# jramapuram/BYOL

Hardware: NVIDIA H100
Metric: images/sec (higher is better)
Workload: dtype bf16

## Files before the change

### byol_b200/csrc/common.cuh

```cuda
#pragma once
#include <cuda.h>
#include <cuda_bf16.h>
#include <cuda_runtime.h>
#include <stdint.h>

namespace byol {

typedef __nv_bfloat16 bf16;

void set_last_error(const char* fmt, ...);
int check_launch(const char* what);

static constexpr int kMaxDevices = 64;
int device_slot();
int device_sm_count();

int smem_opt_in(const void* kernel, int bytes, const char* what);

int tmap_bf16(CUtensorMap* tm, const void* base, int rank, const uint64_t* dims, const uint64_t* byte_strides,
              const uint32_t* box, CUtensorMapSwizzle swizzle, const char* what);
int tmap_2d(CUtensorMap* tm, const void* base, uint64_t rows, uint64_t cols, uint64_t ld, uint32_t box_rows,
            uint32_t box_cols, const char* what);

struct Fix128 {
// ... 74 lines not shown
      ::byol::set_last_error(__VA_ARGS__);        \
      return -1;                                  \
    }                                             \
  } while (0)

__device__ __forceinline__ uint32_t smem_u32(const void* p) {
  return (uint32_t)__cvta_generic_to_shared(p);
}

__device__ __forceinline__ bool elect_one() {
  uint32_t pred = 0;
  asm volatile(
      "{\n"
      ".reg .b32 %%rx;\n"
      ".reg .pred %%px;\n"
      "elect.sync %%rx|%%px, %1;\n"
      "@%%px mov.s32 %0, 1;\n"
      "}\n"
      : "+r"(pred)
      : "r"(0xffffffffu));
  return pred != 0;
}

__device__ __forceinline__ void nesterov_update(float& w, float& buf, float& grad, float lr, float wd, float mu) {
  const float g = __fadd_rn(grad, __fmul_rn(wd, w));
  buf = __fadd_rn(__fmul_rn(mu, buf), g);
  const float d = __fadd_rn(g, __fmul_rn(mu, buf));
  w = __fsub_rn(w, __fmul_rn(lr, d));
  grad = 0.f;
}

__device__ __forceinline__ float warp_sum(float v) {
#pragma unroll
  for (int o = 16; o > 0; o >>= 1) v += __shfl_xor_sync(0xffffffffu, v, o);
  return v;
}

__device__ __forceinline__ void mbar_init(uint64_t* bar, uint32_t count) {
  asm volatile("mbarrier.init.shared::cta.b64 [%0], %1;" ::"r"(smem_u32(bar)), "r"(count) : "memory");
}
__device__ __forceinline__ void fence_mbar_init() {
  asm volatile("fence.mbarrier_init.release.cluster;" ::: "memory");
}
__device__ __forceinline__ void mbar_arrive(uint64_t* bar) {
  asm volatile("mbarrier.arrive.shared::cta.b64 _, [%0];" ::"r"(smem_u32(bar)) : "memory");
}
__device__ __forceinline__ void mbar_arrive_expect_tx(uint64_t* bar, uint32_t bytes) {
  asm volatile("mbarrier.arrive.expect_tx.shared::cta.b64 _, [%0], %1;" ::"r"(smem_u32(bar)), "r"(bytes)
               : "memory");
}
__device__ __forceinline__ bool mbar_try_wait(uint64_t* bar, uint32_t parity) {
  uint32_t ok;
  asm volatile(
      "{\n"
      ".reg .pred p;\n"
      "mbarrier.try_wait.parity.shared::cta.b64 p, [%1], %2;\n"
      "selp.u32 %0, 1, 0, p;\n"
      "}\n"
      : "=r"(ok)
      : "r"(smem_u32(bar)), "r"(parity)
      : "memory");
  return ok != 0;
}
__device__ __forceinline__ void mbar_wait(uint64_t* bar, uint32_t parity) {
  uint32_t spins = 0;
  while (!mbar_try_wait(bar, parity)) {
    if (++spins > (1u << 28)) __trap();
  }
}

__device__ __forceinline__ void fence_proxy_async_smem() {
  asm volatile("fence.proxy.async.shared::cta;" ::: "memory");
}

__device__ __forceinline__ void cp_async16_zfill(uint32_t dst_smem, const void* src, bool valid) {
  uint32_t sz = valid ? 16u : 0u;
  asm volatile("cp.async.cg.shared.global [%0], [%1], 16, %2;" ::"r"(dst_smem), "l"(src), "r"(sz) : "memory");
}
__device__ __forceinline__ void cp_async_commit() { asm volatile("cp.async.commit_group;" ::: "memory"); }
template <int N>
__device__ __forceinline__ void cp_async_wait() {
  asm volatile("cp.async.wait_group %0;" ::"n"(N) : "memory");
}

__device__ __forceinline__ void tma_prefetch_desc(const CUtensorMap* tmap) {
  asm volatile("prefetch.tensormap [%0];" ::"l"(tmap) : "memory");
}
__device__ __forceinline__ void tma_load_2d(uint32_t dst_smem, const CUtensorMap* tmap, uint64_t* bar, int c0,
                                            int c1) {
  asm volatile(
      "cp.async.bulk.tensor.2d.shared::cluster.global.mbarrier::complete_tx::bytes [%0], [%1, {%3, %4}], [%2];"
      ::"r"(dst_smem), "l"(tmap), "r"(smem_u32(bar)), "r"(c0), "r"(c1)
      : "memory");
}

__device__ __forceinline__ void tma_store_2d(const CUtensorMap* tmap, uint32_t src_smem, int c0, int c1) {
  asm volatile("cp.async.bulk.tensor.2d.global.shared::cta.bulk_group [%0, {%2, %3}], [%1];" ::"l"(tmap),
               "r"(src_smem), "r"(c0), "r"(c1)
               : "memory");
}
__device__ __forceinline__ void tma_store_commit() { asm volatile("cp.async.bulk.commit_group;" ::: "memory"); }
__device__ __forceinline__ void tma_store_wait_read() {
  asm volatile("cp.async.bulk.wait_group.read 0;" ::: "memory");
}
__device__ __forceinline__ void tma_store_wait_read1() {
  asm volatile("cp.async.bulk.wait_group.read 1;" ::: "memory");
}
__device__ __forceinline__ void tma_store_wait_all() { asm volatile("cp.async.bulk.wait_group 0;" ::: "memory"); }

__device__ __forceinline__ void wg_fence() { asm volatile("wgmma.fence.sync.aligned;" ::: "memory"); }
__device__ __forceinline__ void wg_commit() { asm volatile("wgmma.commit_group.sync.aligned;" ::: "memory"); }
template <int N>
__device__ __forceinline__ void wg_wait() {
  asm volatile("wgmma.wait_group.sync.aligned %0;" ::"n"(N) : "memory");
}
template <int R>
__device__ __forceinline__ void wg_fence_acc(float (&d)[R]) {
#pragma unroll
  for (int i = 0; i < R; ++i) asm volatile("" : "+f"(d[i])::"memory");
}

template <int N, int TA, int TB>
__device__ __forceinline__ void wgmma_bf16(float (&d)[N / 2], uint64_t adesc, uint64_t bdesc, uint32_t accumulate) {
  static_assert(N == 32 || N == 64 || N == 128 || N == 192 || N == 256, "wgmma_bf16: unsupported N");
  if constexpr (N == 32) {
    asm volatile(
        "{\n.reg .pred p;\nsetp.ne.b32 p, %18, 0;\n"
        "wgmma.mma_async.sync.aligned.m64n32k16.f32.bf16.bf16 {%0, %1, %2, %3, %4, %5, %6, %7, %8, %9, %10, %11, %12, %13, %14, %15}, %16, %17, p, 1, 1, %19, %20;\n}\n"
        : "+f"(d[0]), "+f"(d[1]), "+f"(d[2]), "+f"(d[3]), "+f"(d[4]), "+f"(d[5]), "+f"(d[6]), "+f"(d[7]), "+f"(d[8]), "+f"(d[9]), "+f"(d[10]), "+f"(d[11]), "+f"(d[12]), "+f"(d[13]), "+f"(d[14]), "+f"(d[15])
        : "l"(adesc), "l"(bdesc), "r"(accumulate), "n"(TA), "n"(TB));
  }
  if constexpr (N == 64) {
    asm volatile(
        "{\n.reg .pred p;\nsetp.ne.b32 p, %34, 0;\n"
        "wgmma.mma_async.sync.aligned.m64n64k16.f32.bf16.bf16 {%0, %1, %2, %3, %4, %5, %6, %7, %8, %9, %10, %11, %12, %13, %14, %15, %16, %17, %18, %19, %20, %21, %22, %23, %24, %25, %26, %27, %28, %29, %30, %31}, %32, %33, p, 1, 1, %35, %36;\n}\n"
        : "+f"(d[0]), "+f"(d[1]), "+f"(d[2]), "+f"(d[3]), "+f"(d[4]), "+f"(d[5]), "+f"(d[6]), "+f"(d[7]), "+f"(d[8]), "+f"(d[9]), "+f"(d[10]), "+f"(d[11]), "+f"(d[12]), "+f"(d[13]), "+f"(d[14]), "+f"(d[15]), "+f"(d[16]), "+f"(d[17]), "+f"(d[18]), "+f"(d[19]), "+f"(d[20]), "+f"(d[21]), "+f"(d[22]), "+f"(d[23]), "+f"(d[24]), "+f"(d[25]), "+f"(d[26]), "+f"(d[27]), "+f"(d[28]), "+f"(d[29]), "+f"(d[30]), "+f"(d[31])
        : "l"(adesc), "l"(bdesc), "r"(accumulate), "n"(TA), "n"(TB));
  }
  if constexpr (N == 128) {
    asm volatile(
        "{\n.reg .pred p;\nsetp.ne.b32 p, %66, 0;\n"
        "wgmma.mma_async.sync.aligned.m64n128k16.f32.bf16.bf16 {%0, %1, %2, %3, %4, %5, %6, %7, %8, %9, %10, %11, %12, %13, %14, %15, %16, %17, %18, %19, %20, %21, %22, %23, %24, %25, %26, %27, %28, %29, %30, %31, %32, %33, %34, %35, %36, %37, %38, %39, %40, %41, %42, %43, %44, %45, %46, %47, %48, %49, %50, %51, %52, %53, %54, %55, %56, %57, %58, %59, %60, %61, %62, %63}, %64, %65, p, 1, 1, %67, %68;\n}\n"
        : "+f"(d[0]), "+f"(d[1]), "+f"(d[2]), "+f"(d[3]), "+f"(d[4]), "+f"(d[5]), "+f"(d[6]), "+f"(d[7]), "+f"(d[8]), "+f"(d[9]), "+f"(d[10]), "+f"(d[11]), "+f"(d[12]), "+f"(d[13]), "+f"(d[14]), "+f"(d[15]), "+f"(d[16]), "+f"(d[17]), "+f"(d[18]), "+f"(d[19]), "+f"(d[20]), "+f"(d[21]), "+f"(d[22]), "+f"(d[23]), "+f"(d[24]), "+f"(d[25]), "+f"(d[26]), "+f"(d[27]), "+f"(d[28]), "+f"(d[29]), "+f"(d[30]), "+f"(d[31]), "+f"(d[32]), "+f"(d[33]), "+f"(d[34]), "+f"(d[35]), "+f"(d[36]), "+f"(d[37]), "+f"(d[38]), "+f"(d[39]), "+f"(d[40]), "+f"(d[41]), "+f"(d[42]), "+f"(d[43]), "+f"(d[44]), "+f"(d[45]), "+f"(d[46]), "+f"(d[47]), "+f"(d[48]), "+f"(d[49]), "+f"(d[50]), "+f"(d[51]), "+f"(d[52]), "+f"(d[53]), "+f"(d[54]), "+f"(d[55]), "+f"(d[56]), "+f"(d[57]), "+f"(d[58]), "+f"(d[59]), "+f"(d[60]), "+f"(d[61]), "+f"(d[62]), "+f"(d[63])
        : "l"(adesc), "l"(bdesc), "r"(accumulate), "n"(TA), "n"(TB));
  }
  if constexpr (N == 192) {
    asm volatile(
        "{\n.reg .pred p;\nsetp.ne.b32 p, %98, 0;\n"
        "wgmma.mma_async.sync.aligned.m64n192k16.f32.bf16.bf16 {%0, %1, %2, %3, %4, %5, %6, %7, %8, %9, %10, %11, %12, %13, %14, %15, %16, %17, %18, %19, %20, %21, %22, %23, %24, %25, %26, %27, %28, %29, %30, %31, %32, %33, %34, %35, %36, %37, %38, %39, %40, %41, %42, %43, %44, %45, %46, %47, %48, %49, %50, %51, %52, %53, %54, %55, %56, %57, %58, %59, %60, %61, %62, %63, %64, %65, %66, %67, %68, %69, %70, %71, %72, %73, %74, %75, %76, %77, %78, %79, %80, %81, %82, %83, %84, %85, %86, %87, %88, %89, %90, %91, %92, %93, %94, %95}, %96, %97, p, 1, 1, %99, %100;\n}\n"
        : "+f"(d[0]), "+f"(d[1]), "+f"(d[2]), "+f"(d[3]), "+f"(d[4]), "+f"(d[5]), "+f"(d[6]), "+f"(d[7]), "+f"(d[8]), "+f"(d[9]), "+f"(d[10]), "+f"(d[11]), "+f"(d[12]), "+f"(d[13]), "+f"(d[14]), "+f"(d[15]), "+f"(d[16]), "+f"(d[17]), "+f"(d[18]), "+f"(d[19]), "+f"(d[20]), "+f"(d[21]), "+f"(d[22]), "+f"(d[23]), "+f"(d[24]), "+f"(d[25]), "+f"(d[26]), "+f"(d[27]), "+f"(d[28]), "+f"(d[29]), "+f"(d[30]), "+f"(d[31]), "+f"(d[32]), "+f"(d[33]), "+f"(d[34]), "+f"(d[35]), "+f"(d[36]), "+f"(d[37]), "+f"(d[38]), "+f"(d[39]), "+f"(d[40]), "+f"(d[41]), "+f"(d[42]), "+f"(d[43]), "+f"(d[44]), "+f"(d[45]), "+f"(d[46]), "+f"(d[47]), "+f"(d[48]), "+f"(d[49]), "+f"(d[50]), "+f"(d[51]), "+f"(d[52]), "+f"(d[53]), "+f"(d[54]), "+f"(d[55]), "+f"(d[56]), "+f"(d[57]), "+f"(d[58]), "+f"(d[59]), "+f"(d[60]), "+f"(d[61]), "+f"(d[62]), "+f"(d[63]), "+f"(d[64]), "+f"(d[65]), "+f"(d[66]), "+f"(d[67]), "+f"(d[68]), "+f"(d[69]), "+f"(d[70]), "+f"(d[71]), "+f"(d[72]), "+f"(d[73]), "+f"(d[74]), "+f"(d[75]), "+f"(d[76]), "+f"(d[77]), "+f"(d[78]), "+f"(d[79]), "+f"(d[80]), "+f"(d[81]), "+f"(d[82]), "+f"(d[83]), "+f"(d[84]), "+f"(d[85]), "+f"(d[86]), "+f"(d[87]), "+f"(d[88]), "+f"(d[89]), "+f"(d[90]), "+f"(d[91]), "+f"(d[92]), "+f"(d[93]), "+f"(d[94]), "+f"(d[95])
        : "l"(adesc), "l"(bdesc), "r"(accumulate), "n"(TA), "n"(TB));
  }
  if constexpr (N == 256) {
    asm volatile(
        "{\n.reg .pred p;\nsetp.ne.b32 p, %130, 0;\n"
        "wgmma.mma_async.sync.aligned.m64n256k16.f32.bf16.bf16 {%0, %1, %2, %3, %4, %5, %6, %7, %8, %9, %10, %11, %12, %13, %14, %15, %16, %17, %18, %19, %20, %21, %22, %23, %24, %25, %26, %27, %28, %29, %30, %31, %32, %33, %34, %35, %36, %37, %38, %39, %40, %41, %42, %43, %44, %45, %46, %47, %48, %49, %50, %51, %52, %53, %54, %55, %56, %57, %58, %59, %60, %61, %62, %63, %64, %65, %66, %67, %68, %69, %70, %71, %72, %73, %74, %75, %76, %77, %78, %79, %80, %81, %82, %83, %84, %85, %86, %87, %88, %89, %90, %91, %92, %93, %94, %95, %96, %97, %98, %99, %100, %101, %102, %103, %104, %105, %106, %107, %108, %109, %110, %111, %112, %113, %114, %115, %116, %117, %118, %119, %120, %121, %122, %123, %124, %125, %126, %127}, %128, %129, p, 1, 1, %131, %132;\n}\n"
        : "+f"(d[0]), "+f"(d[1]), "+f"(d[2]), "+f"(d[3]), "+f"(d[4]), "+f"(d[5]), "+f"(d[6]), "+f"(d[7]), "+f"(d[8]), "+f"(d[9]), "+f"(d[10]), "+f"(d[11]), "+f"(d[12]), "+f"(d[13]), "+f"(d[14]), "+f"(d[15]), "+f"(d[16]), "+f"(d[17]), "+f"(d[18]), "+f"(d[19]), "+f"(d[20]), "+f"(d[21]), "+f"(d[22]), "+f"(d[23]), "+f"(d[24]), "+f"(d[25]), "+f"(d[26]), "+f"(d[27]), "+f"(d[28]), "+f"(d[29]), "+f"(d[30]), "+f"(d[31]), "+f"(d[32]), "+f"(d[33]), "+f"(d[34]), "+f"(d[35]), "+f"(d[36]), "+f"(d[37]), "+f"(d[38]), "+f"(d[39]), "+f"(d[40]), "+f"(d[41]), "+f"(d[42]), "+f"(d[43]), "+f"(d[44]), "+f"(d[45]), "+f"(d[46]), "+f"(d[47]), "+f"(d[48]), "+f"(d[49]), "+f"(d[50]), "+f"(d[51]), "+f"(d[52]), "+f"(d[53]), "+f"(d[54]), "+f"(d[55]), "+f"(d[56]), "+f"(d[57]), "+f"(d[58]), "+f"(d[59]), "+f"(d[60]), "+f"(d[61]), "+f"(d[62]), "+f"(d[63]), "+f"(d[64]), "+f"(d[65]), "+f"(d[66]), "+f"(d[67]), "+f"(d[68]), "+f"(d[69]), "+f"(d[70]), "+f"(d[71]), "+f"(d[72]), "+f"(d[73]), "+f"(d[74]), "+f"(d[75]), "+f"(d[76]), "+f"(d[77]), "+f"(d[78]), "+f"(d[79]), "+f"(d[80]), "+f"(d[81]), "+f"(d[82]), "+f"(d[83]), "+f"(d[84]), "+f"(d[85]), "+f"(d[86]), "+f"(d[87]), "+f"(d[88]), "+f"(d[89]), "+f"(d[90]), "+f"(d[91]), "+f"(d[92]), "+f"(d[93]), "+f"(d[94]), "+f"(d[95]), "+f"(d[96]), "+f"(d[97]), "+f"(d[98]), "+f"(d[99]), "+f"(d[100]), "+f"(d[101]), "+f"(d[102]), "+f"(d[103]), "+f"(d[104]), "+f"(d[105]), "+f"(d[106]), "+f"(d[107]), "+f"(d[108]), "+f"(d[109]), "+f"(d[110]), "+f"(d[111]), "+f"(d[112]), "+f"(d[113]), "+f"(d[114]), "+f"(d[115]), "+f"(d[116]), "+f"(d[117]), "+f"(d[118]), "+f"(d[119]), "+f"(d[120]), "+f"(d[121]), "+f"(d[122]), "+f"(d[123]), "+f"(d[124]), "+f"(d[125]), "+f"(d[126]), "+f"(d[127])
        : "l"(adesc), "l"(bdesc), "r"(accumulate), "n"(TA), "n"(TB));
  }
}

template <int N>
__device__ __forceinline__ void acc_store_smem(float* buf, int ld, int row0, int col0, const float (&d)[N / 2]) {
  const int t = threadIdx.x & 127;
  const int r = row0 + (t >> 5) * 16 + ((t & 31) >> 2);
  const int c = col0 + 2 * (t & 3);
// ... 130 lines not shown
```

### byol_b200/csrc/conv_igemm.cu

```cuda
#include <stdarg.h>
#include <stdio.h>
#include <stdlib.h>
#include <string.h>

#include "common.cuh"

namespace byol {

static constexpr int BM = 128;
static constexpr int BK = 64;
static constexpr int A_STAGE_BYTES = BM * 128;
static constexpr int GATHER_LAG = 2;

struct ConvGemmParams {
  const bf16* src;
  void* dst;
  const bf16* resid;
  const uint8_t* resid_mask;
  int resid_up;
  const float* resid_f32;
  const float* bias;
  float* col_sum;
  float* col_sqsum;
  Fix128* fx;
  int Nimg, Hs, Ws, C;
  int Ho, Wo;
  int KH, KW;
  int mul, base, dk, div;
  int M, Ndim, Kg;
  int ldc;
  int num_kb;
  int tiles_n;
  int out_fp32;
  int relu;
  int small_src;
  int local_stats;
  int fold;
  int parity;
  int Hh, Wh;
  int Mc;
  int ncls;
  int cls_list[4];
};

struct TileInfo {
  int m0, n0, nkb;
  int cls_idx, ph, pw, kh0, kw0, nkw;
};

template <bool GROUPED = false>
__device__ __forceinline__ TileInfo tile_info(const ConvGemmParams& p, int tile, int BN_) {
  TileInfo t;
  t.m0 = (tile / p.tiles_n) * BM;
  t.n0 = (tile % p.tiles_n) * BN_;
  t.nkb = p.num_kb;
  t.cls_idx = 0; t.ph = 0; t.pw = 0; t.kh0 = 0; t.kw0 = 0; t.nkw = p.KW;
  if (p.parity) {
    t.cls_idx = t.m0 / p.Mc;
    const int cls = p.cls_list[t.cls_idx];
    t.ph = cls >> 1;
    t.pw = cls & 1;
    t.kh0 = (t.ph + p.base) & 1;
    t.kw0 = (t.pw + p.base) & 1;
    const int nkh = (p.KH - t.kh0 + 1) >> 1;
    t.nkw = (p.KW - t.kw0 + 1) >> 1;
    t.nkb = nkh * t.nkw * (GROUPED ? 1 : p.C / BK);
  }
  return t;
}

template <int BN, int STAGES, bool A_TMA, bool H16 = false>
struct SmemLayout {
  static constexpr int EW = A_TMA ? 8 : 4;
  static constexpr int CPW = (BN / 32) / (EW / 4);
  static constexpr int NBUF = (A_TMA && BN == 128) ? 1 : 2;
  static constexpr int STAGE_PER_WARP = NBUF * 2048;
  static constexpr int B_STAGE_BYTES = BN * 128;
  static constexpr int A_OFF = 0;
  static constexpr int B_OFF = STAGES * A_STAGE_BYTES;
  static constexpr int STAGE_OUT_OFF = B_OFF + STAGES * B_STAGE_BYTES;
  static constexpr int ACC_LD = acc_ld(BN);
  static constexpr int ACC_OFF = STAGE_OUT_OFF + EW * STAGE_PER_WARP;
  static constexpr int OUT_TILE_BYTES = BM * BN * 2;
  static constexpr int BAR_OFF = H16 ? STAGE_OUT_OFF + 2 * OUT_TILE_BYTES : ACC_OFF + BM * ACC_LD * 4;
  static constexpr int NEEDED = BAR_OFF + 256;
  static constexpr int TOTAL = NEEDED + 768;
  static_assert(TOTAL <= 232448, "one CTA per SM: <= 227 KB of dynamic shared memory");
};

static constexpr int IG_THREADS = 17 * 32;

__device__ __forceinline__ void epilogue_bar_sync(int n) { asm volatile("bar.sync 1, %0;" ::"r"(n) : "memory"); }

template <int BN, int STAGES, bool A_TMA, bool GROUPED = false, bool H16 = false>
__global__ void __launch_bounds__(IG_THREADS, 1)
// ... 206 lines not shown
          if (mvalid) {
            float* op = reinterpret_cast<float*>(p.dst) + (int64_t)m * p.ldc + nbase;
            const bool vec = (p.ldc & 3) == 0;
#pragma unroll
            for (int j = 0; j < 32; j += 4) {
              if (vec && nbase + j + 3 < p.Ndim) {
                *reinterpret_cast<float4*>(op + j) = make_float4(v[j], v[j + 1], v[j + 2], v[j + 3]);
              } else {
#pragma unroll
                for (int e = 0; e < 4; ++e)
                  if (nbase + j + e < p.Ndim) op[j + e] = v[j + e];
              }
            }
          }
        } else {
          const uint32_t stage_base = stage_base0 + (uint32_t)sbuf * 2048u;
          if (lane == 0) { if (L::NBUF == 2) tma_store_wait_read1(); else tma_store_wait_read(); }
          __syncwarp();
#pragma unroll
          for (int j = 0; j < 4; ++j) {
            uint4 q;
            q.x = pack_bf16x2(v[8 * j + 0], v[8 * j + 1]);
            q.y = pack_bf16x2(v[8 * j + 2], v[8 * j + 3]);
            q.z = pack_bf16x2(v[8 * j + 4], v[8 * j + 5]);
            q.w = pack_bf16x2(v[8 * j + 6], v[8 * j + 7]);
            const uint32_t off = (uint32_t)lane * 64u + (uint32_t)((j ^ ((lane >> 1) & 3)) << 4);
            asm volatile("st.shared.v4.b32 [%0], {%1, %2, %3, %4};" ::"r"(stage_base + off), "r"(q.x), "r"(q.y),
                         "r"(q.z), "r"(q.w)
                         : "memory");
          }
          fence_proxy_async_smem();
          __syncwarp();
          if (lane == 0) {
            tma_store_2d(&tmapC, stage_base, nbase, mrow0);
            tma_store_commit();
          }
          if (do_stats) stats_narrow(stage_base, lane, rows_valid, cs1[cl], cs2[cl]);
          if (L::NBUF == 2) sbuf ^= 1;
        }
      }
    }
    if (do_stats && stat_n0 >= 0) flush_stats();
    if (local_stats) {
      epilogue_bar_sync(EW * 32);
      for (int i = threadIdx.x; i < 2 * p.Ndim; i += EW * 32) {
        const unsigned long long lo = lstats[2 * i], hi = lstats[2 * i + 1];
        if ((lo | hi) != 0ull) fix_add_words(p.fx + i, lo, (long long)hi);
      }
    }
    if (lane == 0) tma_store_wait_all();
  } else if (!A_TMA && warp >= EW && warp < EW + 4) {
    const int tid = threadIdx.x - 128;
    const int chunk = tid & 7;
    const int row0 = tid >> 3;
    int it = 0;
    const bool fast = GROUPED || ((p.C % BK == 0) && (p.KH * p.KW <= 32) && p.small_src);
    for (int tile = blockIdx.x; tile < num_tiles; tile += gridDim.x) {
      const TileInfo ti = tile_info<GROUPED>(p, tile, BN);
      const int m0 = ti.m0;
      if (!GROUPED && p.fold) {
        uint32_t mask[8];
        int roff[8];
#pragma unroll
        for (int i = 0; i < 8; ++i) {
          const int m = m0 + row0 + 16 * i;
          mask[i] = 0u;
          roff[i] = 0;
          if (m < p.M) {
            const int ow = m % p.Wo;
            const int t = m / p.Wo;
            const int oh = t % p.Ho;
            const int n = t / p.Ho;
            const int bh = oh * p.mul + p.base, bw = ow * p.mul + p.base;
            const int sw = bw + chunk;
            roff[i] = ((n * p.Hs + bh) * p.Ws + sw) * 8;
            if (chunk < p.KW && sw >= 0 && sw < p.Ws)
              for (int kh = 0; kh < p.KH; ++kh)
                if (bh + kh >= 0 && bh + kh < p.Hs) mask[i] |= 1u << kh;
          }
        }
        for (int kb = 0; kb < num_kb; ++kb, ++it) {
          const int s = it % STAGES;
          const uint32_t ph = (it / STAGES) & 1;
          if (it >= GATHER_LAG) {
            cp_async_wait<GATHER_LAG - 1>();
            fence_proxy_async_smem();
            mbar_arrive(&full_bar[(it - GATHER_LAG) % STAGES]);
          }
          mbar_wait(&empty_bar[s], ph ^ 1);
          const int tapoff = kb * p.Ws * 8;
          const uint32_t stage_base = smem_u32(smemA + s * A_STAGE_BYTES);
#pragma unroll
          for (int i = 0; i < 8; ++i) {
            const bool v = (mask[i] >> kb) & 1u;
            const bf16* g = v ? p.src + (roff[i] + tapoff) : p.src;
            cp_async16_zfill(stage_base + sw128_offset(row0 + 16 * i, chunk), g, v);
          }
          cp_async_commit();
        }
      } else if (p.parity) {
        uint32_t mask[8];
        int roff[8];
#pragma unroll
        for (int i = 0; i < 8; ++i) {
          const int mc = m0 + row0 + 16 * i - ti.cls_idx * p.Mc;
          const int b = mc % p.Wh;
          const int t2 = mc / p.Wh;
          const int a = t2 % p.Hh;
          const int n = t2 / p.Hh;
          roff[i] = ((n * p.Hs + a) * p.Ws + b) * p.C;
          mask[i] = 0u;
          int tapi = 0;
          for (int kh = ti.kh0; kh < p.KH; kh += 2)
            for (int kw = ti.kw0; kw < p.KW; kw += 2, ++tapi) {
              const int sh = a + ((ti.ph + p.base - kh) >> 1), sw = b + ((ti.pw + p.base - kw) >> 1);
              if (sh >= 0 && sh < p.Hs && sw >= 0 && sw < p.Ws) mask[i] |= 1u << tapi;
            }
        }
        int kh = ti.kh0, kw = ti.kw0, cc = GROUPED ? ti.n0 : 0, tapi = 0;
        for (int kb = 0; kb < ti.nkb; ++kb, ++it) {
          const int s = it % STAGES;
          const uint32_t ph = (it / STAGES) & 1;
          if (it >= GATHER_LAG) {
            cp_async_wait<GATHER_LAG - 1>();
            fence_proxy_async_smem();
            mbar_arrive(&full_bar[(it - GATHER_LAG) % STAGES]);
          }
          mbar_wait(&empty_bar[s], ph ^ 1);
          const int tapoff = (((ti.ph + p.base - kh) >> 1) * p.Ws + ((ti.pw + p.base - kw) >> 1)) * p.C + cc + chunk * 8;
          const uint32_t stage_base = smem_u32(smemA + s * A_STAGE_BYTES);
#pragma unroll
          for (int i = 0; i < 8; ++i) {
            const bool v = (mask[i] >> tapi) & 1u;
            const bf16* g = v ? p.src + (roff[i] + tapoff) : p.src;
            cp_async16_zfill(stage_base + sw128_offset(row0 + 16 * i, chunk), g, v);
          }
          cp_async_commit();
          if (!GROUPED) cc += BK;
          if (GROUPED || cc >= p.C) {
            if (!GROUPED) cc = 0;
            ++tapi;
            kw += 2;
            if (kw >= p.KW) { kw = ti.kw0; kh += 2; }
          }
        }
      } else if (fast) {
        uint32_t mask[8];
        int roff[8];
#pragma unroll
        for (int i = 0; i < 8; ++i) {
          const int m = m0 + row0 + 16 * i;
          mask[i] = 0u;
          roff[i] = 0;
          if (m < p.M) {
            const int ow = m % p.Wo;
            const int t = m / p.Wo;
            const int oh = t % p.Ho;
            const int n = t / p.Ho;
            const int bh = oh * p.mul + p.base, bw = ow * p.mul + p.base;
            const int sft = p.div == 2 ? 1 : 0;
            roff[i] = ((n * p.Hs + (bh >> sft)) * p.Ws + (bw >> sft)) * p.C;
            int tapi = 0;
            for (int kh = 0; kh < p.KH; ++kh)
              for (int kw = 0; kw < p.KW; ++kw, ++tapi) {
                int sh = bh + kh * p.dk, sw = bw + kw * p.dk;
                bool ok = sh >= 0 && sw >= 0;
                if (p.div == 2) { ok = ok && ((sh | sw) & 1) == 0; sh >>= 1; sw >>= 1; }
                if (ok && sh < p.Hs && sw < p.Ws) mask[i] |= 1u << tapi;
              }
          }
        }
        int kh = 0, kw = 0, cc = GROUPED ? ti.n0 : 0, tapi = 0;
        for (int kb = 0; kb < num_kb; ++kb, ++it) {
          const int s = it % STAGES;
          const uint32_t ph = (it / STAGES) & 1;
          if (it >= GATHER_LAG) {
            cp_async_wait<GATHER_LAG - 1>();
            fence_proxy_async_smem();
            mbar_arrive(&full_bar[(it - GATHER_LAG) % STAGES]);
          }
          mbar_wait(&empty_bar[s], ph ^ 1);
          const int tapoff = (p.div == 2 ? -((kh >> 1) * p.Ws + (kw >> 1)) : (kh * p.Ws + kw) * p.dk) * p.C + cc +
                             chunk * 8;
          const uint32_t stage_base = smem_u32(smemA + s * A_STAGE_BYTES);
#pragma unroll
          for (int i = 0; i < 8; ++i) {
            const bool v = (mask[i] >> tapi) & 1u;
            const bf16* g = v ? p.src + (roff[i] + tapoff) : p.src;
            cp_async16_zfill(stage_base + sw128_offset(row0 + 16 * i, chunk), g, v);
          }
          cp_async_commit();
          if (!GROUPED) cc += BK;
          if (GROUPED || cc >= p.C) {
            if (!GROUPED) cc = 0;
            ++tapi;
            if (++kw == p.KW) { kw = 0; ++kh; }
          }
        }
      } else if (!GROUPED) {
        int bh[8], bw[8];
        int64_t ioff[8];
#pragma unroll
        for (int i = 0; i < 8; ++i) {
          int m = m0 + row0 + 16 * i;
          if (m < p.M) {
            int ow = m % p.Wo;
            int t = m / p.Wo;
            int oh = t % p.Ho;
            int n = t / p.Ho;
            bh[i] = oh * p.mul + p.base;
            bw[i] = ow * p.mul + p.base;
            ioff[i] = (int64_t)n * p.Hs * p.Ws * p.C;
          } else {
            bh[i] = -(1 << 28);
            bw[i] = -(1 << 28);
            ioff[i] = 0;
          }
        }
        for (int kb = 0; kb < num_kb; ++kb, ++it) {
          const int s = it % STAGES;
          const uint32_t ph = (it / STAGES) & 1;
          if (it >= GATHER_LAG) {
            cp_async_wait<GATHER_LAG - 1>();
            fence_proxy_async_smem();
            mbar_arrive(&full_bar[(it - GATHER_LAG) % STAGES]);
          }
          mbar_wait(&empty_bar[s], ph ^ 1);
          const int k0 = kb * BK + chunk * 8;
          const bool kvalid = k0 < p.Kg;
          const int tap = k0 / p.C;
          const int cc = k0 - tap * p.C;
          const int kh = tap / p.KW;
          const int kw = tap - kh * p.KW;
          const int dh = kh * p.dk, dw = kw * p.dk;
          const uint32_t stage_base = smem_u32(smemA + s * A_STAGE_BYTES);
#pragma unroll
          for (int i = 0; i < 8; ++i) {
            int sh = bh[i] + dh, sw = bw[i] + dw;
            bool v = kvalid && sh >= 0 && sw >= 0;
            if (p.div == 2) {
              v = v && ((sh | sw) & 1) == 0;
              sh >>= 1;
              sw >>= 1;
            }
            v = v && sh < p.Hs && sw < p.Ws;
            const bf16* g = v ? p.src + ioff[i] + ((int64_t)sh * p.Ws + sw) * p.C + cc : p.src;
            cp_async16_zfill(stage_base + sw128_offset(row0 + 16 * i, chunk), g, v);
          }
          cp_async_commit();
        }
      }
    }
    cp_async_wait<0>();
    fence_proxy_async_smem();
    for (int j = (it > GATHER_LAG ? it - GATHER_LAG : 0); j < it; ++j) mbar_arrive(&full_bar[j % STAGES]);
  } else if (warp >= MMA_WARP && warp < TMA_WARP) {
    const int wg = (warp - MMA_WARP) >> 2;
    const bool leader = (threadIdx.x & 127) == 0;
    float d[BN / 2];
    int it = 0, local = 0;
    for (int tile = blockIdx.x; tile < num_tiles; tile += gridDim.x, ++local) {
      const int nkb_tile = tile_info<GROUPED>(p, tile, BN).nkb;
      int prev_s = -1;
      for (int kb = 0; kb < nkb_tile; ++kb, ++it) {
        const int s = it % STAGES;
        const uint32_t ph = (it / STAGES) & 1;
        mbar_wait(&full_bar[s], ph);
        const uint64_t adesc = make_smem_desc_sw128(smem_u32(smemA + s * A_STAGE_BYTES + wg * 8192), 16, 1024);
        const uint64_t bdesc = make_smem_desc_sw128(smem_u32(smemB + s * L::B_STAGE_BYTES), 16, 1024);
        wg_fence();
#pragma unroll
        for (int k = 0; k < BK / 16; ++k) {
          wgmma_bf16<BN, 0, 0>(d, adesc + (uint64_t)(2 * k), bdesc + (uint64_t)(2 * k), (uint32_t)((kb | k) != 0));
        }
        wg_commit();
        wg_wait<1>();
        if (leader && prev_s >= 0) mbar_arrive(&empty_bar[prev_s]);
        prev_s = s;
      }
      wg_wait<0>();
      wg_fence_acc(d);
      if (leader && prev_s >= 0) mbar_arrive(&empty_bar[prev_s]);
      if constexpr (H16) {
        const int buf = local & 1;
        mbar_wait(&oempty_bar[buf], (uint32_t)(((local >> 1) & 1) ^ 1));
        acc_store_bf16_sw64<BN>(smem_u32(stage_out + buf * L::OUT_TILE_BYTES) + (uint32_t)wg * 2 * (BN / 32) * 2048u, d);
        fence_proxy_async_smem();
        mbar_arrive(&ofull_bar[buf]);
      } else {
        mbar_wait(tempty_bar, (uint32_t)((local & 1) ^ 1));
        acc_store_smem<BN>(accbuf, L::ACC_LD, wg * 64, 0, d);
        mbar_arrive(tfull_bar);
      }
    }
  } else if (warp == TMA_WARP) {
    if (lane == 0) {
      constexpr uint32_t tx = (uint32_t)L::B_STAGE_BYTES + (A_TMA ? (uint32_t)A_STAGE_BYTES : 0u);
      int it = 0;
      for (int tile = blockIdx.x; tile < num_tiles; tile += gridDim.x) {
        const TileInfo ti = tile_info<GROUPED>(p, tile, BN);
        const int n0 = ti.n0;
        const int m0 = ti.m0;
        int kh = ti.kh0, kw = ti.kw0, cc = 0;
        for (int kb = 0; kb < ti.nkb; ++kb, ++it) {
          const int s = it % STAGES;
          const uint32_t ph = (it / STAGES) & 1;
          mbar_wait(&empty_bar[s], ph ^ 1);
          mbar_arrive_expect_tx(&full_bar[s], tx);
          int kcol = kb * BK;
          if (p.parity) {
            kcol = (kh * p.KW + kw) * (GROUPED ? BK : p.C) + cc;
            if (!GROUPED) cc += BK;
            if (GROUPED || cc >= p.C) { cc = 0; kw += 2; if (kw >= p.KW) { kw = ti.kw0; kh += 2; } }
          }
          tma_load_2d(smem_u32(smemB + s * L::B_STAGE_BYTES), &tmapB, &full_bar[s], kcol, n0);
          if (A_TMA) tma_load_2d(smem_u32(smemA + s * A_STAGE_BYTES), &tmapA, &full_bar[s], kb * BK, m0);
        }
      }
    }
    __syncwarp();
  }
}

struct WgradParams {
  const bf16* src;
  float* dw;
  int Nimg, Hs, Ws, C;
  int Ho, Wo;
  int KH, KW;
  int stride, pad;
  int M;
  int Cout, Cin_real;
  int tiles_co, tiles_n;
  int splits, kb_per_split, num_kb_total;
  int Cg;
  int groups;
  int fold_kw;
  int small_src;
  float* part;
  int64_t ndw;
  int terms, kb_per_term;
  int ldsrc;
  int dy_term;
  int src_term[6];
};

static constexpr int WG_KROWS = 64;
static constexpr int WG_A_STAGE = 2 * WG_KROWS * 128;

static constexpr int WG_THREADS = 13 * 32;

template <int BN, int STAGES, bool B_TMA, bool GROUPED = false>
__global__ void __launch_bounds__(WG_THREADS, 1)
conv_wgrad_kernel(const __grid_constant__ CUtensorMap tmapA, const __grid_constant__ CUtensorMap tmapB,
                  const WgradParams p) {
  static_assert(!GROUPED || (BN == 128 && !B_TMA), "grouped mode: two 64-channel chunks, gathered B operand");
  constexpr int NCH = BN / 64;
  constexpr int NMMA = GROUPED ? 64 : BN;
  constexpr int B_STAGE = NCH * WG_KROWS * 128;
  extern __shared__ uint8_t smem_raw[];
  uint8_t* smem = (uint8_t*)(((uintptr_t)smem_raw + 1023) & ~(uintptr_t)1023);
  uint8_t* smemA = smem;
  uint8_t* smemB = smem + STAGES * WG_A_STAGE;
  uint64_t* full_bar = (uint64_t*)(smemB + STAGES * B_STAGE);
  uint64_t* empty_bar = full_bar + STAGES;

  const int warp = __shfl_sync(0xffffffffu, (int)(threadIdx.x >> 5), 0);
  const int lane = threadIdx.x & 31;
  int bid = blockIdx.x;
  const int tile_n = bid % p.tiles_n;    bid /= p.tiles_n;
  const int tile_co = bid % p.tiles_co;  bid /= p.tiles_co;
  const int split = bid;
  const int co0 = tile_co * 128;
  const int n0 = tile_n * BN;
  const int kb_begin = split * p.kb_per_split;
  int kb_end = kb_begin + p.kb_per_split;
  if (kb_end > p.num_kb_total) kb_end = p.num_kb_total;
  const int nkb = kb_end - kb_begin;
  const int taps = p.KH * p.KW;

  if (warp == 12 && lane == 0) {
    for (int s = 0; s < STAGES; ++s) {
      mbar_init(&full_bar[s], B_TMA ? 1u : 129u);
      mbar_init(&empty_bar[s], 2u);
    }
    fence_mbar_init();
    tma_prefetch_desc(&tmapA);
    if (B_TMA) tma_prefetch_desc(&tmapB);
  }
  __syncthreads();

  if (warp < 4) {
    if (!B_TMA) {
      constexpr int CHUNKS = NCH * 8;
      constexpr int PER_THREAD = WG_KROWS * CHUNKS / 128;
      const int chunk = threadIdx.x % CHUNKS;
      const int rbase = (threadIdx.x / CHUNKS) * PER_THREAD;
      const int ch64 = chunk >> 3, c16 = chunk & 7;
      const int col = n0 + chunk * 8;
      const int group = col / p.Cg;
      const int cw = col - group * p.Cg;
      int kh, kw, ci;
      bool cvalid = group < p.groups;
      if (p.fold_kw) { kh = group; kw = cw >> 3; ci = 0; cvalid = cvalid && kw < p.KW; }
      else           { kh = group / p.KW; kw = group - kh * p.KW; ci = cw; }
      if (GROUPED) { ci += co0; cvalid = cvalid && ci < p.C; }
      const int dh = kh - p.pad, dw = kw - p.pad;
      const int64_t sC = (int64_t)p.stride * p.ldsrc;
      for (int it = 0; it < nkb; ++it) {
        const int kb = kb_begin + it;
        const int term = p.terms == 1 ? 0 : kb / p.kb_per_term;
        const int s = it % STAGES;
        const uint32_t ph = (it / STAGES) & 1;
        if (it >= GATHER_LAG) {
          cp_async_wait<GATHER_LAG - 1>();
          fence_proxy_async_smem();
          mbar_arrive(&full_bar[(it - GATHER_LAG) % STAGES]);
        }
        mbar_wait(&empty_bar[s], ph ^ 1);
        const uint32_t stage_base = smem_u32(smemB + s * B_STAGE) + ch64 * (WG_KROWS * 128);
        const int cterm = ci + p.src_term[term];
        int m = (kb - term * p.kb_per_term) * WG_KROWS + rbase;
        int ow = m % p.Wo;
        int t = m / p.Wo;
        int oh = t % p.Ho;
        int n = t / p.Ho;
        int sw = ow * p.stride + dw;
        int sh = oh * p.stride + dh;
        bool hvalid = cvalid && sh >= 0 && sh < p.Hs;
        int64_t off = (((int64_t)n * p.Hs + sh) * p.Ws + sw) * p.ldsrc + cterm;
#pragma unroll
        for (int i = 0; i < PER_THREAD; ++i) {
          const bool v = hvalid && m < p.M && sw >= 0 && sw < p.Ws;
          cp_async16_zfill(stage_base + sw128_offset(rbase + i, c16), v ? p.src + off : p.src, v);
          ++m;
          sw += p.stride;
          off += sC;
          if (++ow == p.Wo) {
            ow = 0;
            if (++oh == p.Ho) { oh = 0; ++n; }
            sw = dw;
            sh = oh * p.stride + dh;
            hvalid = cvalid && sh >= 0 && sh < p.Hs;
            off = (((int64_t)n * p.Hs + sh) * p.Ws + sw) * p.ldsrc + cterm;
          }
        }
        cp_async_commit();
      }
      cp_async_wait<0>();
      fence_proxy_async_smem();
      for (int it = (nkb > GATHER_LAG ? nkb - GATHER_LAG : 0); it < nkb; ++it) mbar_arrive(&full_bar[it % STAGES]);
    }
  } else if (warp < 12) {
    const int wg = (warp - 4) >> 2;
    const bool leader = (threadIdx.x & 127) == 0;
    float d[NMMA / 2];
    int prev_s = -1;
    for (int it = 0; it < nkb; ++it) {
      const int s = it % STAGES;
      const uint32_t ph = (it / STAGES) & 1;
      mbar_wait(&full_bar[s], ph);
      const uint64_t adesc =
          make_smem_desc_sw128(smem_u32(smemA + s * WG_A_STAGE + wg * WG_KROWS * 128), WG_KROWS * 128, 1024);
      const uint64_t bdesc = make_smem_desc_sw128(
          smem_u32(smemB + s * B_STAGE + (GROUPED ? wg * WG_KROWS * 128 : 0)), WG_KROWS * 128, 1024);
      wg_fence();
#pragma unroll
      for (int k = 0; k < WG_KROWS / 16; ++k) {
        wgmma_bf16<NMMA, 1, 1>(d, adesc + (uint64_t)(128 * k), bdesc + (uint64_t)(128 * k), (uint32_t)((it | k) != 0));
      }
      wg_commit();
      wg_wait<1>();
      if (leader && prev_s >= 0) mbar_arrive(&empty_bar[prev_s]);
      prev_s = s;
    }
    wg_wait<0>();
    wg_fence_acc(d);
    const int t = threadIdx.x & 127;
    const int r0 = wg * 64 + (t >> 5) * 16 + ((t & 31) >> 2);
    float* const part = p.part != nullptr ? p.part + (int64_t)split * p.ndw : nullptr;
    auto add = [&](float* q, float v) {
      if (part != nullptr) part[q - p.dw] = v;
      else wgrad_add_single(q, v);
    };
    if (GROUPED) {
      const int gs = p.Cin_real;
      const int tap = n0 / BN;
#pragma unroll
      for (int j = 0; j < NMMA / 8; ++j) {
#pragma unroll
        for (int h = 0; h < 2; ++h) {
          const int co = co0 + r0 + 8 * h;
          if (co >= p.Cout) continue;
#pragma unroll
          for (int e = 0; e < 2; ++e) {
            const int ci = co0 + wg * 64 + 8 * j + 2 * (t & 3) + e;
            if (co / gs == ci / gs) add(p.dw + ((int64_t)co * gs + ci % gs) * taps + tap, d[4 * j + 2 * h + e]);
          }
        }
      }
      return;
    }
#pragma unroll
    for (int j = 0; j < BN / 8; ++j) {
#pragma unroll
      for (int h = 0; h < 2; ++h) {
        const int co = co0 + r0 + 8 * h;
        const int colb = n0 + 8 * j + 2 * (t & 3);
        const int group = colb / p.Cg;
        const int cw = colb - group * p.Cg;
        const float v0 = d[4 * j + 2 * h], v1 = d[4 * j + 2 * h + 1];
        if (co >= p.Cout || group >= p.groups) continue;
        if (p.fold_kw) {
          float* gp = p.dw + ((int64_t)co * p.Cin_real) * taps + group * p.KW;
#pragma unroll
          for (int e = 0; e < 2; ++e) {
            const int kwj = (cw + e) >> 3, cj = (cw + e) & 7;
            if (kwj < p.KW && cj < p.Cin_real) add(gp + (int64_t)cj * taps + kwj, e ? v1 : v0);
          }
        } else {
          float* gp = p.dw + ((int64_t)co * p.Cin_real) * taps + group;
          if (cw < p.Cin_real) add(gp + (int64_t)cw * taps, v0);
          if (cw + 1 < p.Cin_real) add(gp + (int64_t)(cw + 1) * taps, v1);
        }
      }
    }
  } else {
    if (lane == 0) {
      constexpr uint32_t tx = (uint32_t)WG_A_STAGE + (B_TMA ? (uint32_t)B_STAGE : 0u);
      for (int it = 0; it < nkb; ++it) {
        const int kb = kb_begin + it;
        const int term = p.terms == 1 ? 0 : kb / p.kb_per_term;
        const int row = (kb - term * p.kb_per_term) * WG_KROWS;
        const int col_a = co0 + term * p.dy_term;
        const int s = it % STAGES;
        const uint32_t ph = (it / STAGES) & 1;
        mbar_wait(&empty_bar[s], ph ^ 1);
        mbar_arrive_expect_tx(&full_bar[s], tx);
        const uint32_t a_base = smem_u32(smemA + s * WG_A_STAGE);
        tma_load_2d(a_base, &tmapA, &full_bar[s], col_a, row);
        tma_load_2d(a_base + WG_KROWS * 128, &tmapA, &full_bar[s], col_a + 64, row);
        if (B_TMA) {
          const uint32_t b_base = smem_u32(smemB + s * B_STAGE);
#pragma unroll
// ... 136 lines not shown
  }
  if (a_tma) {
    if (tmap_2d(&ta, src, (uint64_t)p.M, (uint64_t)C, (uint64_t)C, (uint32_t)BM, 64u, "conv_igemm A") != 0) return -3;
  } else {
    ta = tb;
  }
  if (col_sum != nullptr) {
    p.fx = fix_scratch(stream, 2 * (int64_t)Ndim);
    if (p.fx == nullptr) return -2;
  }
  int rc;
  if (grouped) {
    rc = launch_igemm<64, 4, false, true>(ta, tb, tc, p, tiles_m, stream);
  } else if (BN == 128) {
    rc = h16     ? launch_igemm<128, 3, true, false, true>(ta, tb, tc, p, tiles_m, stream)
         : a_tma ? launch_igemm<128, 3, true>(ta, tb, tc, p, tiles_m, stream)
                 : launch_igemm<128, 3, false>(ta, tb, tc, p, tiles_m, stream);
  } else {
    rc = h16     ? launch_igemm<64, 3, true, false, true>(ta, tb, tc, p, tiles_m, stream)
         : a_tma ? launch_igemm<64, 3, true>(ta, tb, tc, p, tiles_m, stream)
                 : launch_igemm<64, 4, false>(ta, tb, tc, p, tiles_m, stream);
  }
  if (rc != 0 || col_sum == nullptr) return rc;
  return fix_flush_stats(p.fx, col_sum, col_sqsum, Ndim, stream);
}

extern "C" int byol_conv_igemm(const void* src, const void* wt, void* dst, const void* resid,
                               const void* resid_mask, int resid_up, const float* bias, float* col_sum, float* col_sqsum, int Nimg, int Hs, int Ws, int C, int Ho, int Wo,
                               int Ndim, int KH, int KW, int stride, int pad, int mode, int ldw, int ldc,
                               int out_fp32, int relu, int force_gather, cudaStream_t stream) {
  return conv_igemm_impl(src, wt, dst, resid, nullptr, resid_mask, resid_up, bias, col_sum, col_sqsum, Nimg, Hs, Ws, C,
                         Ho, Wo, Ndim, KH, KW, stride, pad, mode, ldw, ldc, out_fp32, relu, force_gather, stream);
}

static bool grouped_geometry_ok(const char* what, int Nimg, int H, int W, int C, int Ho, int Wo, int KH, int KW,
                                int stride, int pad) {
  if (Nimg <= 0 || H <= 0 || W <= 0 || C < 64 || C % 64 != 0 || KH != 3 || KW != 3 || pad != 1 ||
      (stride != 1 && stride != 2) || Ho != (H - 1) / stride + 1 || Wo != (W - 1) / stride + 1) {
    set_last_error("%s: unsupported geometry (N=%d H=%d W=%d C=%d Ho=%d Wo=%d KH=%d KW=%d stride=%d pad=%d): needs "
                   "C %% 64 == 0, 3x3, pad 1, stride 1 or 2", what, Nimg, H, W, C, Ho, Wo, KH, KW, stride, pad);
    return false;
  }
  const int64_t big = (int64_t)Nimg * (H > Ho ? H : Ho) * (W > Wo ? W : Wo) * C;
  if (big >= (1ll << 31) - (1ll << 24)) {
    set_last_error("%s: tensor of %lld elements too large for 32-bit offsets", what, (long long)big);
    return false;
  }
  return true;
}

extern "C" int byol_conv_fprop_grouped(const void* x, const void* wt, void* y, float* col_sum, float* col_sqsum,
                                       int Nimg, int H, int W, int C, int Ho, int Wo, int KH, int KW, int stride,
                                       int pad, cudaStream_t stream) {
  BYOL_CHECK_ARG(x && wt && y, "byol_conv_fprop_grouped: null pointer");
  if (!grouped_geometry_ok("byol_conv_fprop_grouped", Nimg, H, W, C, Ho, Wo, KH, KW, stride, pad)) return -1;
  return conv_igemm_impl(x, wt, y, nullptr, nullptr, nullptr, 0, nullptr, col_sum, col_sqsum, Nimg, H, W, C, Ho, Wo,
                         C, KH, KW, stride, pad, 0, KH * KW * BK, C, 0, 0, 0, stream, 1);
}

extern "C" int byol_conv_dgrad_grouped(const void* dy, const void* wd, void* dx, int Nimg, int Ho, int Wo, int C,
                                       int H, int W, int KH, int KW, int stride, int pad, cudaStream_t stream) {
  BYOL_CHECK_ARG(dy && wd && dx, "byol_conv_dgrad_grouped: null pointer");
  if (!grouped_geometry_ok("byol_conv_dgrad_grouped", Nimg, H, W, C, Ho, Wo, KH, KW, stride, pad)) return -1;
  return conv_igemm_impl(dy, wd, dx, nullptr, nullptr, nullptr, 0, nullptr, nullptr, nullptr, Nimg, Ho, Wo, C, H, W,
                         C, KH, KW, stride, pad, 1, KH * KW * BK, C, 0, 0, 0, stream, 1);
}

extern "C" int byol_conv_dgrad_planes(const void* dy, const void* wd, float* dx, const float* resid_f32, int Nimg,
                                      int Hs, int Ws, int Cout, int H, int W, int Cin, int KH, int KW, int stride,
                                      int pad, int T, cudaStream_t stream) {
  BYOL_CHECK_ARG((T == 3 || T == 6) && Cout % 8 == 0 && Cin % 8 == 0, "byol_conv_dgrad_planes: bad args (T=%d Cout=%d Cin=%d)",
                 T, Cout, Cin);
  return conv_igemm_impl(dy, wd, dx, nullptr, resid_f32, nullptr, 0, nullptr, nullptr, nullptr, Nimg, Hs, Ws, T * Cout,
                         H, W, Cin, KH, KW, stride, pad, 1, KH * KW * T * Cout, Cin, 1, 0, 0, stream);
}

template <int BN, bool B_TMA, bool GROUPED = false>
static int launch_wgrad(const CUtensorMap& ta, const CUtensorMap& tb, const WgradParams& p, int grid,
                        cudaStream_t stream) {
  constexpr int STAGES = 4;
  constexpr int SMEM = STAGES * (WG_A_STAGE + (BN / 64) * WG_KROWS * 128) + 256 + 1024;
  auto kern = conv_wgrad_kernel<BN, STAGES, B_TMA, GROUPED>;
  if (smem_opt_in((const void*)kern, SMEM, "conv_wgrad_kernel") != 0) return -2;
  kern<<<grid, WG_THREADS, SMEM, stream>>>(ta, tb, p);
  return check_launch("conv_wgrad_kernel");
}

static int conv_wgrad_impl(const void* src, const void* dy, float* dw, int Nimg, int Hs, int Ws, int C, int Cin_real,
                           int Ho, int Wo, int Cout, int ldy, int KH, int KW, int stride, int pad, int force_gather,
                           int T, cudaStream_t stream, int gs = 0) {
  BYOL_CHECK_ARG(src && dy && dw, "byol_conv_wgrad: null pointer");
  if (ldy == 0) ldy = Cout;
  if (gs > 0) {
    if (!force_gather && Hs == Ho && Ws == Wo && patch_wgrad_applicable(Hs, Ws, C, C, Cout, KH, KW, stride, pad))
      return patch_wgrad_launch(src, dy, dw, Nimg, Hs, Ws, C, Cout, device_sm_count(), stream, gs);
  }
  BYOL_CHECK_ARG(C % 8 == 0 && ldy % 8 == 0 && ldy >= Cout && Cout > 0,
                 "byol_conv_wgrad: C=%d and the dy pitch %d must be multiples of 8 (Cout=%d)", C, ldy, Cout);
  BYOL_CHECK_ARG(Cin_real <= C, "byol_conv_wgrad: Cin_real > C");
  BYOL_CHECK_ARG(T == 0 || T == 3 || T == 6, "byol_conv_wgrad: bad T=%d", T);
  const int64_t M64 = (int64_t)Nimg * Ho * Wo;
  BYOL_CHECK_ARG(M64 > 0 && M64 < (1ll << 31), "byol_conv_wgrad: M out of range");
  if (T == 0 && !force_gather && ldy == Cout && Hs == Ho && Ws == Wo && patch_wgrad_applicable(Hs, Ws, C, Cin_real, Cout, KH, KW, stride, pad))
    return patch_wgrad_launch(src, dy, dw, Nimg, Hs, Ws, C, Cout, device_sm_count(), stream);
  const int terms = T == 0 ? 1 : T;
  WgradParams p;
  memset(&p, 0, sizeof(p));
  p.terms = terms;
  p.ldsrc = C * terms;
  p.dy_term = ldy;
  const int perm3[3] = {0, 2, 1}, perm6[6] = {0, 2, 1, 3, 5, 4};
  for (int j = 0; j < terms; ++j) p.src_term[j] = (T == 3 ? perm3[j] : T == 6 ? perm6[j] : 0) * C;
  p.src = (const bf16*)src;
  p.dw = dw;
  p.Nimg = Nimg; p.Hs = Hs; p.Ws = Ws; p.C = C; p.Ho = Ho; p.Wo = Wo; p.KH = KH; p.KW = KW;
  p.stride = stride; p.pad = pad;
  p.M = (int)M64;
  p.Cout = Cout;
  p.Cin_real = Cin_real;
  p.fold_kw = (C == 8 && KW <= 8 && KW > 1) ? 1 : 0;
  BYOL_CHECK_ARG(p.fold_kw || C % 64 == 0 || KH * KW == 1, "byol_conv_wgrad: C=%d must be 8 (stem) or a multiple of 64", C);
  p.Cg = p.fold_kw ? 64 : gs > 0 ? 128 : C;
  p.groups = p.fold_kw ? KH : KH * KW;
  const int ncols = p.groups * p.Cg;
  const int BN = ncols > 64 ? 128 : 64;
  p.tiles_co = (Cout + 127) / 128;
  p.tiles_n = (ncols + BN - 1) / BN;
  p.kb_per_term = (p.M + WG_KROWS - 1) / WG_KROWS;
  p.num_kb_total = terms * p.kb_per_term;
  p.small_src = ((int64_t)Nimg * Hs * Ws * p.ldsrc < (1ll << 31) - (1ll << 24)) ? 1 : 0;
  const int taps = KH * KW;
  const int base_ctas = p.tiles_co * p.tiles_n;
  const int target_ctas = device_sm_count();
  int splits = target_ctas / base_ctas;
  int max_splits = (p.num_kb_total + 7) / 8;
  if (max_splits < 1) max_splits = 1;
  if (splits > max_splits) splits = max_splits;
  if (splits < 1) splits = 1;
  p.kb_per_split = (p.num_kb_total + splits - 1) / splits;
  p.splits = (p.num_kb_total + p.kb_per_split - 1) / p.kb_per_split;
  const int grid = base_ctas * p.splits;
  const bool b_tma = !force_gather && KH == 1 && KW == 1 && stride == 1 && pad == 0;

  BYOL_CHECK_ARG(!b_tma || C % 8 == 0, "byol_conv_wgrad: bad C");
  CUtensorMap ta, tb;
  const uint64_t dy_cols = T == 0 ? (uint64_t)Cout : (uint64_t)terms * ldy;
  if (tmap_2d(&ta, dy, (uint64_t)p.M, dy_cols, (uint64_t)terms * ldy, (uint32_t)WG_KROWS, 64u, "conv_wgrad dY") != 0)
    return -3;
  if (b_tma) {
    if (tmap_2d(&tb, src, (uint64_t)p.M, (uint64_t)p.ldsrc, (uint64_t)p.ldsrc, (uint32_t)WG_KROWS, 64u, "conv_wgrad X") != 0)
      return -3;
  } else {
    tb = ta;
  }
  p.ndw = (int64_t)Cout * Cin_real * taps;
  if (p.splits > 1) {
    p.part = part_scratch(stream, p.splits * p.ndw);
    if (p.part == nullptr) return -2;
  }
  const int rc = gs > 0 ? launch_wgrad<128, false, true>(ta, tb, p, grid, stream)
               : BN == 128 ? (b_tma ? launch_wgrad<128, true>(ta, tb, p, grid, stream) : launch_wgrad<128, false>(ta, tb, p, grid, stream))
                           : (b_tma ? launch_wgrad<64, true>(ta, tb, p, grid, stream) : launch_wgrad<64, false>(ta, tb, p, grid, stream));
  if (rc != 0 || p.splits == 1) return rc;
  return wgrad_reduce(p.part, p.splits, dw, p.ndw, stream);
}

extern "C" int byol_conv_wgrad_grouped(const void* x, const void* dy, float* dw, int Nimg, int H, int W, int C, int Cg,
// ... 21 lines not shown
```

Before: 2516.

## Signal gather completion via cp.async mbarrier arrive and widen wgrad gather warps

New measurement: 2549 (median of 6 runs). 1.01x the previous value.

```diff
diff --git a/byol_b200/csrc/common.cuh b/byol_b200/csrc/common.cuh
--- a/byol_b200/csrc/common.cuh
+++ b/byol_b200/csrc/common.cuh
@@ -180,6 +180,10 @@
 __device__ __forceinline__ void cp_async_wait() {
   asm volatile("cp.async.wait_group %0;" ::"n"(N) : "memory");
 }
+__device__ __forceinline__ void cp_async_wait_all() { asm volatile("cp.async.wait_all;" ::: "memory"); }
+__device__ __forceinline__ void cp_async_mbar_arrive(uint64_t* bar) {
+  asm volatile("cp.async.mbarrier.arrive.noinc.shared::cta.b64 [%0];" ::"r"(smem_u32(bar)) : "memory");
+}
 
 __device__ __forceinline__ void tma_prefetch_desc(const CUtensorMap* tmap) {
   asm volatile("prefetch.tensormap [%0];" ::"l"(tmap) : "memory");
diff --git a/byol_b200/csrc/conv_igemm.cu b/byol_b200/csrc/conv_igemm.cu
--- a/byol_b200/csrc/conv_igemm.cu
+++ b/byol_b200/csrc/conv_igemm.cu
@@ -10,7 +10,6 @@
 static constexpr int BM = 128;
 static constexpr int BK = 64;
 static constexpr int A_STAGE_BYTES = BM * 128;
-static constexpr int GATHER_LAG = 2;
 
 struct ConvGemmParams {
   const bf16* src;
@@ -383,11 +382,6 @@
         for (int kb = 0; kb < num_kb; ++kb, ++it) {
           const int s = it % STAGES;
           const uint32_t ph = (it / STAGES) & 1;
-          if (it >= GATHER_LAG) {
-            cp_async_wait<GATHER_LAG - 1>();
-            fence_proxy_async_smem();
-            mbar_arrive(&full_bar[(it - GATHER_LAG) % STAGES]);
-          }
           mbar_wait(&empty_bar[s], ph ^ 1);
           const int tapoff = kb * p.Ws * 8;
           const uint32_t stage_base = smem_u32(smemA + s * A_STAGE_BYTES);
@@ -397,7 +391,7 @@
             const bf16* g = v ? p.src + (roff[i] + tapoff) : p.src;
             cp_async16_zfill(stage_base + sw128_offset(row0 + 16 * i, chunk), g, v);
           }
-          cp_async_commit();
+          cp_async_mbar_arrive(&full_bar[s]);
         }
       } else if (p.parity) {
         uint32_t mask[8];
@@ -422,11 +416,6 @@
         for (int kb = 0; kb < ti.nkb; ++kb, ++it) {
           const int s = it % STAGES;
           const uint32_t ph = (it / STAGES) & 1;
-          if (it >= GATHER_LAG) {
-            cp_async_wait<GATHER_LAG - 1>();
-            fence_proxy_async_smem();
-            mbar_arrive(&full_bar[(it - GATHER_LAG) % STAGES]);
-          }
           mbar_wait(&empty_bar[s], ph ^ 1);
           const int tapoff = (((ti.ph + p.base - kh) >> 1) * p.Ws + ((ti.pw + p.base - kw) >> 1)) * p.C + cc + chunk * 8;
           const uint32_t stage_base = smem_u32(smemA + s * A_STAGE_BYTES);
@@ -436,7 +425,7 @@
             const bf16* g = v ? p.src + (roff[i] + tapoff) : p.src;
             cp_async16_zfill(stage_base + sw128_offset(row0 + 16 * i, chunk), g, v);
           }
-          cp_async_commit();
+          cp_async_mbar_arrive(&full_bar[s]);
           if (!GROUPED) cc += BK;
           if (GROUPED || cc >= p.C) {
             if (!GROUPED) cc = 0;
@@ -475,11 +464,6 @@
         for (int kb = 0; kb < num_kb; ++kb, ++it) {
           const int s = it % STAGES;
           const uint32_t ph = (it / STAGES) & 1;
-          if (it >= GATHER_LAG) {
-            cp_async_wait<GATHER_LAG - 1>();
-            fence_proxy_async_smem();
-            mbar_arrive(&full_bar[(it - GATHER_LAG) % STAGES]);
-          }
           mbar_wait(&empty_bar[s], ph ^ 1);
           const int tapoff = (p.div == 2 ? -((kh >> 1) * p.Ws + (kw >> 1)) : (kh * p.Ws + kw) * p.dk) * p.C + cc +
                              chunk * 8;
@@ -490,7 +474,7 @@
             const bf16* g = v ? p.src + (roff[i] + tapoff) : p.src;
             cp_async16_zfill(stage_base + sw128_offset(row0 + 16 * i, chunk), g, v);
           }
-          cp_async_commit();
+          cp_async_mbar_arrive(&full_bar[s]);
           if (!GROUPED) cc += BK;
           if (GROUPED || cc >= p.C) {
             if (!GROUPED) cc = 0;
@@ -521,11 +505,6 @@
         for (int kb = 0; kb < num_kb; ++kb, ++it) {
           const int s = it % STAGES;
           const uint32_t ph = (it / STAGES) & 1;
-          if (it >= GATHER_LAG) {
-            cp_async_wait<GATHER_LAG - 1>();
-            fence_proxy_async_smem();
-            mbar_arrive(&full_bar[(it - GATHER_LAG) % STAGES]);
-          }
           mbar_wait(&empty_bar[s], ph ^ 1);
           const int k0 = kb * BK + chunk * 8;
           const bool kvalid = k0 < p.Kg;
@@ -548,13 +527,11 @@
             const bf16* g = v ? p.src + ioff[i] + ((int64_t)sh * p.Ws + sw) * p.C + cc : p.src;
             cp_async16_zfill(stage_base + sw128_offset(row0 + 16 * i, chunk), g, v);
           }
-          cp_async_commit();
-        }
-      }
-    }
-    cp_async_wait<0>();
-    fence_proxy_async_smem();
-    for (int j = (it > GATHER_LAG ? it - GATHER_LAG : 0); j < it; ++j) mbar_arrive(&full_bar[j % STAGES]);
+          cp_async_mbar_arrive(&full_bar[s]);
+        }
+      }
+    }
+    cp_async_wait_all();
   } else if (warp >= MMA_WARP && warp < TMA_WARP) {
     const int wg = (warp - MMA_WARP) >> 2;
     const bool leader = (threadIdx.x & 127) == 0;
@@ -567,6 +544,7 @@
         const int s = it % STAGES;
         const uint32_t ph = (it / STAGES) & 1;
         mbar_wait(&full_bar[s], ph);
+        if (!A_TMA) fence_proxy_async_smem();
         const uint64_t adesc = make_smem_desc_sw128(smem_u32(smemA + s * A_STAGE_BYTES + wg * 8192), 16, 1024);
         const uint64_t bdesc = make_smem_desc_sw128(smem_u32(smemB + s * L::B_STAGE_BYTES), 16, 1024);
         wg_fence();
@@ -575,6 +553,11 @@
           wgmma_bf16<BN, 0, 0>(d, adesc + (uint64_t)(2 * k), bdesc + (uint64_t)(2 * k), (uint32_t)((kb | k) != 0));
         }
         wg_commit();
+        if (!A_TMA) {
+          wg_wait<0>();
+          if (leader) mbar_arrive(&empty_bar[s]);
+          continue;
+        }
         wg_wait<1>();
         if (leader && prev_s >= 0) mbar_arrive(&empty_bar[prev_s]);
         prev_s = s;
@@ -649,10 +632,11 @@
 static constexpr int WG_KROWS = 64;
 static constexpr int WG_A_STAGE = 2 * WG_KROWS * 128;
 
-static constexpr int WG_THREADS = 13 * 32;
+__host__ __device__ constexpr int wg_gather_warps(bool b_tma) { return b_tma ? 4 : 8; }
+__host__ __device__ constexpr int wg_threads(bool b_tma) { return (wg_gather_warps(b_tma) + 9) * 32; }
 
 template <int BN, int STAGES, bool B_TMA, bool GROUPED = false>
-__global__ void __launch_bounds__(WG_THREADS, 1)
+__global__ void __launch_bounds__(wg_threads(B_TMA), 1)
 conv_wgrad_kernel(const __grid_constant__ CUtensorMap tmapA, const __grid_constant__ CUtensorMap tmapB,
                   const WgradParams p) {
   static_assert(!GROUPED || (BN == 128 && !B_TMA), "grouped mode: two 64-channel chunks, gathered B operand");
@@ -680,9 +664,10 @@
   const int nkb = kb_end - kb_begin;
   const int taps = p.KH * p.KW;
 
-  if (warp == 12 && lane == 0) {
+  constexpr int GW = wg_gather_warps(B_TMA);
+  if (warp == GW + 8 && lane == 0) {
     for (int s = 0; s < STAGES; ++s) {
-      mbar_init(&full_bar[s], B_TMA ? 1u : 129u);
+      mbar_init(&full_bar[s], B_TMA ? 1u : (uint32_t)(GW * 32 + 1));
       mbar_init(&empty_bar[s], 2u);
     }
     fence_mbar_init();
@@ -691,10 +676,10 @@
   }
   __syncthreads();
 
-  if (warp < 4) {
+  if (warp < GW) {
     if (!B_TMA) {
       constexpr int CHUNKS = NCH * 8;
-      constexpr int PER_THREAD = WG_KROWS * CHUNKS / 128;
+      constexpr int PER_THREAD = WG_KROWS * CHUNKS / (GW * 32);
       const int chunk = threadIdx.x % CHUNKS;
       const int rbase = (threadIdx.x / CHUNKS) * PER_THREAD;
       const int ch64 = chunk >> 3, c16 = chunk & 7;
@@ -713,13 +698,6 @@
         const int term = p.terms == 1 ? 0 : kb / p.kb_per_term;
         const int s = it % STAGES;
         const uint32_t ph = (it / STAGES) & 1;
-        if (it >= GATHER_LAG) {
-          cp_async_wait<GATHER_LAG - 1>();
-          fence_proxy_async_smem();
-          mbar_arrive(&full_bar[(it - GATHER_LAG) % STAGES]);
-        }
-        mbar_wait(&empty_bar[s], ph ^ 1);
-        const uint32_t stage_base = smem_u32(smemB + s * B_STAGE) + ch64 * (WG_KROWS * 128);
         const int cterm = ci + p.src_term[term];
         int m = (kb - term * p.kb_per_term) * WG_KROWS + rbase;
         int ow = m % p.Wo;
@@ -730,10 +708,13 @@
         int sh = oh * p.stride + dh;
         bool hvalid = cvalid && sh >= 0 && sh < p.Hs;
         int64_t off = (((int64_t)n * p.Hs + sh) * p.Ws + sw) * p.ldsrc + cterm;
+        const bf16* g[PER_THREAD];
+        uint32_t vmask = 0u;
 #pragma unroll
         for (int i = 0; i < PER_THREAD; ++i) {
           const bool v = hvalid && m < p.M && sw >= 0 && sw < p.Ws;
-          cp_async16_zfill(stage_base + sw128_offset(rbase + i, c16), v ? p.src + off : p.src, v);
+          g[i] = v ? p.src + off : p.src;
+          vmask |= (uint32_t)v << i;
           ++m;
           sw += p.stride;
           off += sC;
@@ -746,14 +727,17 @@
             off = (((int64_t)n * p.Hs + sh) * p.Ws + sw) * p.ldsrc + cterm;
           }
         }
-        cp_async_commit();
-      }
-      cp_async_wait<0>();
-      fence_proxy_async_smem();
-      for (int it = (nkb > GATHER_LAG ? nkb - GATHER_LAG : 0); it < nkb; ++it) mbar_arrive(&full_bar[it % STAGES]);
-    }
-  } else if (warp < 12) {
-    const int wg = (warp - 4) >> 2;
+        mbar_wait(&empty_bar[s], ph ^ 1);
+        const uint32_t stage_base = smem_u32(smemB + s * B_STAGE) + ch64 * (WG_KROWS * 128);
+#pragma unroll
+        for (int i = 0; i < PER_THREAD; ++i)
+          cp_async16_zfill(stage_base + sw128_offset(rbase + i, c16), g[i], (vmask >> i) & 1u);
+        cp_async_mbar_arrive(&full_bar[s]);
+      }
+      cp_async_wait_all();
+    }
+  } else if (warp < GW + 8) {
+    const int wg = (warp - GW) >> 2;
     const bool leader = (threadIdx.x & 127) == 0;
     float d[NMMA / 2];
     int prev_s = -1;
@@ -761,6 +745,7 @@
       const int s = it % STAGES;
       const uint32_t ph = (it / STAGES) & 1;
       mbar_wait(&full_bar[s], ph);
+      if (!B_TMA) fence_proxy_async_smem();
       const uint64_t adesc =
           make_smem_desc_sw128(smem_u32(smemA + s * WG_A_STAGE + wg * WG_KROWS * 128), WG_KROWS * 128, 1024);
       const uint64_t bdesc = make_smem_desc_sw128(
@@ -1063,7 +1048,7 @@
   constexpr int SMEM = STAGES * (WG_A_STAGE + (BN / 64) * WG_KROWS * 128) + 256 + 1024;
   auto kern = conv_wgrad_kernel<BN, STAGES, B_TMA, GROUPED>;
   if (smem_opt_in((const void*)kern, SMEM, "conv_wgrad_kernel") != 0) return -2;
-  kern<<<grid, WG_THREADS, SMEM, stream>>>(ta, tb, p);
+  kern<<<grid, wg_threads(B_TMA), SMEM, stream>>>(ta, tb, p);
   return check_launch("conv_wgrad_kernel");
 }
 
```
